# florasion/D-VQVAE

Measured on AMD Instinct MI355X. Metric: grasps/sec at batch=65536, N=1024 pts, K=512, higher is better.
Workload: dtype f32 (GEMMs: every fp32 operand as two fp16 pieces, a1 = fp16(a), a2 = fp16((a - a1) * 2^11), weights pre-scaled by one power of two per output row; the 3 partial products a1 b1, a1 b2, a2 b1 are exact in fp32 and accumulate in TWO fp32 accumulators (large / cross terms) on v_mfma_f32_16x16x32_f16; d

## Files before the change

d-vqvae_amd/_lib.py:

```python
from __future__ import annotations

import ctypes as C
import os
import subprocess
import threading

_HERE = os.path.dirname(os.path.abspath(__file__))
LIB_PATH = os.path.join(_HERE, "libdvq_hip.so")
if os.environ.get("DVQ_DIAG_LIB") == "1":
    LIB_PATH = os.path.join(os.path.dirname(_HERE), "tools", "diag", "libdvq_hip_diag.so")
    print("[dvq] DVQ_DIAG_LIB=1: loading the DIAGNOSTICS build; results are invalid when a DVQ_*_ABL variable is set",
          file=__import__("sys").stderr)
CSRC = os.path.join(_HERE, "csrc")
HEADER = os.path.join(os.path.dirname(_HERE), "include", "dvq.h")

_lock = threading.Lock()
_lib = None

DVQ_MAX_SRC = 8
ABI_VERSION = 10
PLANES_BF16X3, PLANES_F16X2 = 0, 1

c_f32p = C.c_void_p
c_i64p = C.c_void_p
# ... 72 lines not shown
    "dvq_vq_fast_workspace_bytes": (C.c_size_t, [C.c_int64, C.c_int, C.c_int]),
    "dvq_vq_argmin_fast": (C.c_int, [c_f32p, c_f32p, C.c_void_p, C.c_int64, C.c_int, C.c_int, c_i64p, C.c_void_p,
                                     C.c_void_p, C.c_size_t, c_stream]),
    "dvq_vq_lookup": (C.c_int, [c_f32p, c_i64p, C.c_int64, C.c_int64, C.c_int, C.c_int, c_f32p, C.c_int64, c_i32p, c_stream]),
    "dvq_pointnet_workspace_bytes": (C.c_size_t, [C.c_int64, C.c_int]),
    "dvq_pointnet_fault_counters": (C.c_int, [C.POINTER(C.c_uint64), C.c_int]),
    "dvq_pointnet_filter_bytes": (C.c_size_t, []),
    "dvq_pointnet_pack_filter": (C.c_int, [C.c_void_p, C.c_void_p, C.c_void_p, C.c_void_p]),
    "dvq_pointnet_encode": (C.c_int, [C.POINTER(PointnetWeights), c_f32p, C.c_int64, C.c_int, c_f32p, C.c_int64, c_f32p,
                                      C.c_void_p, C.c_size_t, c_stream]),
    "dvq_pixelcnn_tables_bytes": (C.c_size_t, [C.POINTER(PixelcnnWeights)]),
    "dvq_pixelcnn_build_tables": (C.c_int, [C.POINTER(PixelcnnWeights), C.c_void_p, C.c_size_t, c_stream]),
    "dvq_pixelcnn_workspace_bytes": (C.c_size_t, [C.POINTER(PixelcnnWeights), C.c_int64]),
    "dvq_pixelcnn_sample": (C.c_int, [C.POINTER(PixelcnnWeights), c_i64p, c_f32p, C.c_int64, c_i64p, c_f32p, c_i32p,
                                      C.c_void_p, C.c_size_t, c_stream]),
    "dvq_pixelcnn_sample_ctl": (C.c_int, [C.POINTER(PixelcnnWeights), c_i64p, c_f32p, C.c_int64, C.POINTER(PixelcnnCtl), c_i64p, c_f32p,
                                          c_i32p, C.c_void_p, C.c_size_t, c_stream]),
    "dvq_pixelcnn_forward": (C.c_int, [C.POINTER(PixelcnnWeights), c_i64p, c_i64p, C.c_int64, c_f32p, c_i32p, C.c_void_p,
                                       C.c_size_t, c_stream]),
    "dvq_pixelcnn_beam_workspace_bytes": (C.c_size_t, [C.POINTER(PixelcnnWeights), C.c_int64, C.c_int32]),
    "dvq_pixelcnn_beam": (C.c_int, [C.POINTER(PixelcnnWeights), c_i64p, C.c_int64, C.c_int32, c_i64p, c_f32p, c_i32p,
                                    C.POINTER(PixelcnnBeamTrace), c_i32p, C.c_void_p, C.c_size_t, c_stream]),
    "dvq_mano_workspace_bytes": (C.c_size_t, [C.c_int64]),
    "dvq_mano_forward": (C.c_int, [C.POINTER(ManoModel), c_f32p, C.c_int64, c_f32p, C.c_int64, c_f32p, C.c_int64, c_f32p,
                                   C.c_int64, C.c_int64, c_f32p, C.c_int, c_f32p, C.c_void_p, C.c_size_t, c_stream]),
    "dvq_mano_backward_workspace_bytes": (C.c_size_t, [C.c_int64]),
    "dvq_mano_backward": (C.c_int, [C.POINTER(ManoModel), c_f32p, c_f32p, C.c_int64, c_f32p, C.c_int64, c_f32p, C.c_int64, c_f32p,
                                    C.c_int64, C.c_int64, c_f32p, C.c_int, c_f32p, c_f32p, c_f32p, c_f32p, c_f32p, C.c_void_p,
                                    C.c_size_t, c_stream]),
    "dvq_copy_cols": (C.c_int, [c_f32p, C.c_int64, C.c_int64, C.c_int, c_f32p, C.c_int64, c_stream]),
# ... 102 lines not shown
```

d-vqvae_amd/csrc/misc.hip:

```cpp
#include "dvq_internal.h"
#include <string.h>

static thread_local char g_err[512] = "";

void dvq_set_error(const char* fmt, ...) {
    va_list ap;
    va_start(ap, fmt);
    vsnprintf(g_err, sizeof(g_err), fmt, ap);
    va_end(ap);
}

extern "C" const char* dvq_last_error(void) { return g_err; }
extern "C" int dvq_abi_version(void) { return DVQ_ABI_VERSION; }

namespace {
std::mutex g_knob_lock;
std::atomic<const DvqKnobs*> g_knobs{nullptr};
DvqKnobs* read_knobs() {
    DvqKnobs* k = new DvqKnobs();
    auto is = [](const char* name, char c) { const char* e = getenv(name); return e && e[0] == c; };
    auto num = [](const char* name) { const char* e = getenv(name); return e ? atol(e) : 0L; };
    k->gemm_wide = !is("DVQ_GEMM_WIDE", '0');
    k->gemm_tn = (int)num("DVQ_GEMM_TN");
    k->gemm_dephase = !is("DVQ_GEMM_DEPHASE", '0');
// ... 165 lines not shown
    if (b >= B) return;
    const float* src = pc + b * pc_bstride;
    const float x = src[n], y = src[N + n], z = src[2 * N + n];
    const float* r = R + b * 9;
    float* dst = out + b * (long)C * N;
#pragma unroll
    for (int i = 0; i < 3; ++i) {
        float v = r[i * 3 + 0] * x;
        v = fmaf(r[i * 3 + 1], y, v);
        v = fmaf(r[i * 3 + 2], z, v);
        dst[i * N + n] = v + (t ? t[i] : 0.f);
    }
    for (int c = 3; c < C; ++c) dst[c * N + n] = src[c * N + n];
}

__device__ __forceinline__ void philox4x32_10(unsigned (&c)[4], unsigned k0, unsigned k1) {
#pragma unroll
    for (int r = 0; r < 10; ++r) {
        const unsigned long long p0 = (unsigned long long)0xD2511F53u * c[0], p1 = (unsigned long long)0xCD9E8D57u * c[2];
        const unsigned n0 = (unsigned)(p1 >> 32) ^ c[1] ^ k0, n1 = (unsigned)p1, n2 = (unsigned)(p0 >> 32) ^ c[3] ^ k1, n3 = (unsigned)p0;
        c[0] = n0; c[1] = n1; c[2] = n2; c[3] = n3;
        k0 += 0x9E3779B9u;
        k1 += 0xBB67AE85u;
    }
}

__device__ __forceinline__ f32x4 exp1_quad(unsigned long long seed, unsigned stream_id, unsigned long long grow, unsigned q) {
    unsigned c[4] = {q, (unsigned)grow, (unsigned)(grow >> 32), stream_id};
    philox4x32_10(c, (unsigned)seed, (unsigned)(seed >> 32));
    f32x4 v;
#pragma unroll
    for (int i = 0; i < 4; ++i) v[i] = -logf(((float)(c[i] >> 8) + 0.5f) * 5.9604644775390625e-08f);
    return v;
}

__global__ void exp1_noise_kernel(unsigned long long seed, unsigned stream_id, long row0, long rows, int cols, float* __restrict__ out,
                                  const int64_t* __restrict__ perm) {
    const int quads = cols / 4;
    const long gid = (long)blockIdx.x * blockDim.x + threadIdx.x;
    const long r = gid / quads;
    const int q = (int)(gid % quads);
    if (r >= rows) return;
    const unsigned long long grow = (unsigned long long)(row0 + (perm ? (long)perm[r] : r));
    *reinterpret_cast<f32x4*>(out + r * cols + 4 * q) = exp1_quad(seed, stream_id, grow, (unsigned)q);
}

__global__ void exp1_noise_keyed_kernel(unsigned long long seed, const int64_t* __restrict__ stream_ids, const int64_t* __restrict__ row_ids,
                                        long rows, int cols, float* __restrict__ out, int32_t* err_flag) {
    const int quads = cols / 4;
    const long gid = (long)blockIdx.x * blockDim.x + threadIdx.x;
    const long r = gid / quads;
    const int q = (int)(gid % quads);
    if (r >= rows) return;
    const int64_t sid = stream_ids[r], row = row_ids[r];
    f32x4 v;
    if (sid >= 0 && sid <= (int64_t)0xFFFFFFFFLL && row >= 0) {
        v = exp1_quad(seed, (unsigned)sid, (unsigned long long)row, (unsigned)q);
    } else {
        const float nan = __builtin_nanf("");
        v = f32x4{nan, nan, nan, nan};
        if (q == 0 && err_flag) atomicOr(err_flag, 1);
    }
    *reinterpret_cast<f32x4*>(out + r * cols + 4 * q) = v;
}

constexpr int TC_THREADS = 256;
constexpr int TC_SPAN = TC_THREADS * 4;
__device__ __forceinline__ float tc_component(float r0, float r1, float r2, float x, float y, float z, float t) {
    float v = r0 * x;
    v = fmaf(r1, y, v);
    v = fmaf(r2, z, v);
// ... 198 lines not shown
```

d-vqvae_amd/csrc/pixelcnn.hip:

```cpp
#include "dvq_internal.h"

namespace {

constexpr int GRID = 3, NPOS = 9;

__global__ void sanitize_labels_kernel(const int64_t* __restrict__ label, long B, int n_classes, int64_t* __restrict__ out,
                                       int32_t* err_flag) {
    const long b = (long)blockIdx.x * blockDim.x + threadIdx.x;
    if (b >= B) return;
    int64_t l = label[b];
    if (l < 0 || l >= n_classes) {
        if (err_flag) atomicOr(err_flag, 1);
        l = 0;
    }
    out[b] = l;
}

__global__ void bias_gate_kernel(const float* __restrict__ bias, const float* __restrict__ cls, const int64_t* __restrict__ label,
                                 long M, int dim, float* __restrict__ out, float* __restrict__ pre) {
    const long gid = (long)blockIdx.x * blockDim.x + threadIdx.x;
    const long m = gid / dim;
    const int c = (int)(gid % dim);
    if (m >= M) return;
    const int na = (c / 64) * 128 + ((c % 64) / 32) * 64 + (c % 32);
    const int nb = na + 32;
    float a = bias[na], g = bias[nb];
    if (pre) {
        pre[m * 2 * dim + na] = a;
        pre[m * 2 * dim + nb] = g;
    }
    const float* crow = cls + label[m] * 2 * dim;
    a += crow[na];
    g += crow[nb];
    out[m * dim + c] = tanhf(a) * (1.0f / (1.0f + expf(-g)));
}

__global__ void sample_kernel(const float* __restrict__ logits, const float* __restrict__ noise ,
                              int pos, int n_in, long Bc, const int64_t* __restrict__ forced ,
                              int64_t* __restrict__ codes , const float* __restrict__ tok_emb, int dim,
                              float* __restrict__ x0 , float* __restrict__ logits_out ,
                              int32_t* err_flag, const int64_t* __restrict__ lrow ) {
    const int lane = threadIdx.x & 63;
    const long b = (long)blockIdx.x * (blockDim.x >> 6) + (threadIdx.x >> 6);
    if (b >= Bc) return;
    const float* lg = logits + (lrow ? lrow[b] : b) * n_in;
    int64_t code;
    if (logits_out)
        for (int k = lane; k < n_in; k += 64) logits_out[(b * NPOS + pos) * n_in + k] = lg[k];
    if (forced) {
        code = forced[b * NPOS + pos];
        if (code < 0 || code >= n_in) {
            if (lane == 0 && err_flag) atomicOr(err_flag, 1);
            code = 0;
        }
    } else {
        float mx = -INFINITY;
        for (int k = lane; k < n_in; k += 64) mx = fmaxf(mx, lg[k]);
#pragma unroll
        for (int o = 32; o > 0; o >>= 1) mx = fmaxf(mx, __shfl_xor(mx, o));
        float sum = 0.f;
        for (int k = lane; k < n_in; k += 64) sum += expf(lg[k] - mx);
#pragma unroll
        for (int o = 32; o > 0; o >>= 1) sum += __shfl_xor(sum, o);
        const float* q = noise + (b * NPOS + pos) * n_in;
        float best = -INFINITY;
        int bi = 0x7fffffff;
        for (int k = lane; k < n_in; k += 64) {
            const float p = expf(lg[k] - mx) / sum;
            const float s = p / q[k];
            if (s > best || (s == best && k < bi)) { best = s; bi = k; }
        }
#pragma unroll
        for (int o = 32; o > 0; o >>= 1) {
            const float ob = __shfl_xor(best, o);
            const int oi = __shfl_xor(bi, o);
            if (ob > best || (ob == best && oi < bi)) { best = ob; bi = oi; }
        }
        const bool nan_draw = bi == 0x7fffffff;
        if (nan_draw) {
            bi = 0;
            if (lane == 0 && err_flag) atomicOr(err_flag, 4);
        }
        code = bi;
        if (lane == 0) codes[b * NPOS + pos] = nan_draw ? -1 : code;
    }
    const float* e = tok_emb + code * dim;
    for (int c = lane * 4; c < dim; c += 256) *reinterpret_cast<f32x4*>(x0 + b * dim + c) = *reinterpret_cast<const f32x4*>(e + c);
}

__device__ __forceinline__ uint32_t order_key(float v) {
    if (v == 0.f) v = 0.f;
    const uint32_t u = __float_as_uint(v);
    return (u & 0x80000000u) ? ~u : (u | 0x80000000u);
}

__device__ __forceinline__ void row_softmax_stats(const float* __restrict__ lg, int n_in, int lane, float& mx, float& sum) {
    mx = -INFINITY;
    for (int k = lane; k < n_in; k += 64) mx = fmaxf(mx, lg[k]);
#pragma unroll
    for (int o = 32; o > 0; o >>= 1) mx = fmaxf(mx, __shfl_xor(mx, o));
// ... 145 lines not shown
        const float sc = lc / T;
        float lm, ld = code_kept ? (sc - mx) - logf(sum) : -INFINITY;
        if (T == 1.0f && !sel) {
            lm = ld;
        } else {
            float mxl, suml;
            row_softmax_stats(lg, n_in, lane, mxl, suml);
            lm = (lc - mxl) - logf(suml);
        }
        if (nan_row || nan_draw) lm = ld = __builtin_nanf("");
        if (lane == 0) {
            if (logp_model) logp_model[b * NPOS + pos] = lm;
            if (logp_draw) logp_draw[b * NPOS + pos] = ld;
        }
    }
    const float* e = tok_emb + code * dim;
    for (int c = lane * 4; c < dim; c += 256) *reinterpret_cast<f32x4*>(x0 + b * dim + c) = *reinterpret_cast<const f32x4*>(e + c);
}

__global__ void iota_kernel(int64_t* __restrict__ out, int n) {
    const int i = blockIdx.x * blockDim.x + threadIdx.x;
    if (i < n) out[i] = i;
}

__device__ __forceinline__ uint32_t order_key_bits(uint32_t u) {
    if ((u << 1) == 0u) u = 0u;
    return (u & 0x80000000u) ? ~u : (u | 0x80000000u);
}

constexpr int BEAM_MAX_W = 1024, BEAM_THREADS = 1024, BEAM_WAVES = BEAM_THREADS / 64;
// ... 277 lines not shown
int check_weights(const dvq_pixelcnn_weights* w) {
    DVQ_REQUIRE(w && w->layers_host && w->tok_emb && w->w0 && w->b0 && w->w2 && w->b2, "pixelcnn: null weights");
    DVQ_REQUIRE(w->n_layers >= 1 && w->dim >= 64 && w->dim % 64 == 0, "pixelcnn: dim=%d must be a multiple of 64", w->dim);
    DVQ_REQUIRE(w->n_hidden % 32 == 0 && w->n_in >= 1 && w->n_classes >= 1, "pixelcnn: bad head sizes");
    DVQ_REQUIRE(w->planes_kind == DVQ_PLANES_BF16X3 || w->planes_kind == DVQ_PLANES_F16X2, "pixelcnn: unknown planes_kind %d", w->planes_kind);
    if (w->planes_kind == DVQ_PLANES_F16X2 && w->w0_p) {
        DVQ_REQUIRE(w->s0 && w->s2, "pixelcnn: fp16 planes without row scales (head)");
        for (int l = 0; l < w->n_layers; ++l)
            DVQ_REQUIRE(w->layers_host[l].sv && w->layers_host[l].sh && w->layers_host[l].sr, "pixelcnn: fp16 planes without row scales (layer %d)", l);
    }
    return DVQ_OK;
}

int run(const dvq_pixelcnn_weights* w, const int64_t* label, const float* noise, const int64_t* forced, int64_t B,
        int64_t* codes, float* logits_out, int32_t* err_flag, void* ws, size_t ws_bytes, hipStream_t st, void* build = nullptr,
        const dvq_pixelcnn_ctl* ctl = nullptr, const BeamCall* beam = nullptr) {
    DVQ_PROPAGATE(check_weights(w));
    Plan pl;
    if (build) {
        pl = Plan{};
        pl.L = w->n_layers;
        pl.dim = w->dim;
        pl.tab = true;
        (void)carve_tables(pl, w, (char*)build);
    } else {
        DVQ_REQUIRE(B >= 0, "pixelcnn: negative batch");
        if (B == 0) return DVQ_OK;
        DVQ_REQUIRE(label && (beam || forced || (codes && (noise || (ctl && ctl->given)))), "pixelcnn: null input");
        DVQ_REQUIRE(ws && dvq_aligned16(ws), "pixelcnn: null/unaligned workspace");
        pl = make_plan(w, B, ws, beam ? beam->W : 0);
        if (ws_bytes < pl.bytes) {
            dvq_set_error("pixelcnn: workspace %zu < %zu bytes", ws_bytes, pl.bytes);
            return DVQ_EWORKSPACE;
        }
    }
    const int dim = w->dim, L = w->n_layers;
    const int kind = w->planes_kind;

    struct Act { const float* p; const int64_t* arow; };
    auto vertical_layer = [&](int r, int l, long M, const int64_t* lab, auto xv_of ,
                              auto out_of , auto pre_of ,
                              int mode, auto state_of ) -> int {
        const dvq_pixelcnn_layer& ly = w->layers_host[l];
// ... 227 lines not shown
            }
            return Act{pl.XH(level, pos), nullptr};
        };
        for (int r = 0; r < GRID; ++r) {
            cur_r = r;
            cur_pos = r * GRID;
            if (!(pl.tab && r == 0))
                for (int l = 0; l < L; ++l)
                    DVQ_PROPAGATE(vertical_layer(r, l, Bc, pl.lab, xv_b, [&](int c) { return pl.XV(l + 1, r * GRID + c); },
                                                 [&](int c) { return pl.HV(l, c); }, (pl.tab && r == 1 && !beam) ? 2 : 0,
                                                 [&](int c, int which) { return pl.SV(l, c, which); }));
            for (int c = 0; c < GRID; ++c) {
                const int pos = r * GRID + c;
                cur_pos = pos;
                const bool from_table = pl.tab && pos == 0;
                if (!from_table)
                    DVQ_PROPAGATE(horizontal_position(r, c, Bc, pl.lab, [&](int layer, int col) { return hv_b(layer, col, r); }, xh_b,
                                                      [&](int level) { return pl.XH(level, pos); }, pl.g, pl.hid, pl.lg,
                                                      (pl.tab && r == 0 && !beam) ? 2 : 0,
                                                      [&](int layer, int which) { return pl.SH(layer, c, which); }));
                if (beam) {
                    const dvq_pixelcnn_beam_trace* tr = beam->trace;
                    const size_t toff = ((size_t)pos * beam->S + s0) * beam->W;
                    {
                        DVQ_PROF("pixelcnn_beam_score", 0, (double)Bc * 2.0 * w->n_in * 4, st);
                        DVQ_LAUNCH(beam_score_kernel, dim3((unsigned)((Bc + 3) / 4)), dim3(256), 0, st, pl.lg, w->n_in, Bc, beam->W, pl.bscore,
                                   pl.blive, pl.bnan, tr && tr->logits ? tr->logits + toff * w->n_in : nullptr,
                                   from_table ? pl.lgc : nullptr, pl.lab);
                        DVQ_CHECK_LAUNCH("pixelcnn_beam_score");
                    }
// ... 4 lines not shown
                               tr && tr->token ? tr->token + toff : nullptr, tr && tr->score ? tr->score + toff : nullptr,
                               tr && tr->live ? tr->live + (size_t)pos * beam->S + s0 : nullptr);
                    acur ^= 1;
                } else if (ctl) {
                    DVQ_PROF("pixelcnn_draw", 0, (double)Bc * (2.0 * w->n_in + dim) * 4, st);
                    const dim3 grid((unsigned)((Bc + 3) / 4)), block(256);
                    const float* lgp = from_table ? pl.lgc : pl.lg;
                    const float* qp = noise ? noise + b0 * NPOS * w->n_in : nullptr;
                    const int64_t* gp = ctl->given ? ctl->given + b0 * NPOS : nullptr;
                    float* lo = logits_out ? logits_out + b0 * NPOS * w->n_in : nullptr;
                    float* pm = ctl->logp_model_out ? ctl->logp_model_out + b0 * NPOS : nullptr;
                    float* pd = ctl->logp_draw_out ? ctl->logp_draw_out + b0 * NPOS : nullptr;
                    const int64_t* lr = from_table ? pl.lab : nullptr;
                    if (w->n_in <= 512)
                        DVQ_LAUNCH(sample_ctl_kernel<true>, grid, block, 0, st, lgp, qp, pos, w->n_in, Bc, gp, codes + b0 * NPOS, w->tok_emb,
                                   dim, pl.XV(0, pos), lo, err_flag, lr, ctl->temperature, ctl->top_k, pm, pd);
                    else
                        DVQ_LAUNCH(sample_ctl_kernel<false>, grid, block, 0, st, lgp, qp, pos, w->n_in, Bc, gp, codes + b0 * NPOS, w->tok_emb,
                                   dim, pl.XV(0, pos), lo, err_flag, lr, ctl->temperature, ctl->top_k, pm, pd);
                } else {
                DVQ_PROF("pixelcnn_draw", 0, (double)Bc * (2.0 * w->n_in + dim) * 4, st);
                DVQ_LAUNCH(sample_kernel, dim3((unsigned)((Bc + 3) / 4)), dim3(256), 0, st, from_table ? pl.lgc : pl.lg,
                                   noise ? noise + b0 * NPOS * w->n_in : nullptr, pos, w->n_in, Bc,
                                   forced ? forced + b0 * NPOS : nullptr, codes ? codes + b0 * NPOS : nullptr, w->tok_emb, dim,
                                   pl.XV(0, pos), logits_out ? logits_out + b0 * NPOS * w->n_in : nullptr, err_flag,
                                   from_table ? pl.lab : nullptr);
                }
                DVQ_CHECK_LAUNCH("pixelcnn_sample_step");
            }
        }
        if (beam) {
            DVQ_LAUNCH(beam_finish_kernel, dim3((unsigned)((Bc + 255) / 256)), dim3(256), 0, st, pl.btok, pl.anc[acur], pl.chunk, Bc, beam->W,
                       pl.bscore, pl.blive, beam->codes + b0 * NPOS, beam->score + b0, beam->n_live + s0);
            DVQ_CHECK_LAUNCH("pixelcnn_beam_finish");
        }
    }
    return DVQ_OK;
}

}

// ... 9 lines not shown
                "pixelcnn_build_tables: class tables exist for fp16 weight images only (DVQ_PLANES_F16X2)");
    DVQ_REQUIRE(tables_bytes >= dvq_pixelcnn_tables_bytes(w), "pixelcnn_build_tables: buffer %zu < %zu bytes", tables_bytes,
                dvq_pixelcnn_tables_bytes(w));
    return run(w, nullptr, nullptr, nullptr, 0, nullptr, nullptr, nullptr, nullptr, 0, (hipStream_t)stream, tables);
}

extern "C" size_t dvq_pixelcnn_workspace_bytes(const dvq_pixelcnn_weights* w, int64_t B) {
    if (!w || B <= 0) return 256;
    return make_plan(w, B, nullptr).bytes;
}

extern "C" int dvq_pixelcnn_sample(const dvq_pixelcnn_weights* w, const int64_t* label, const float* noise, int64_t B,
                                   int64_t* codes, float* logits_out, int32_t* err_flag, void* workspace,
                                   size_t workspace_bytes, dvq_stream_t stream) {
    return run(w, label, noise, nullptr, B, codes, logits_out, err_flag, workspace, workspace_bytes, (hipStream_t)stream);
}

extern "C" int dvq_pixelcnn_sample_ctl(const dvq_pixelcnn_weights* w, const int64_t* label, const float* noise, int64_t B,
                                       const dvq_pixelcnn_ctl* ctl, int64_t* codes, float* logits_out, int32_t* err_flag,
                                       void* workspace, size_t workspace_bytes, dvq_stream_t stream) {
    DVQ_REQUIRE(ctl, "pixelcnn_sample_ctl: null controls");
    DVQ_REQUIRE(ctl->temperature > 0.f && ctl->temperature <= 3.4028234664e38f, "pixelcnn_sample_ctl: temperature must be finite and > 0");
    DVQ_REQUIRE(ctl->top_k >= 0, "pixelcnn_sample_ctl: top_k must be >= 0 (0: off)");
    DVQ_REQUIRE(codes, "pixelcnn_sample_ctl: null codes");
    return run(w, label, noise, nullptr, B, codes, logits_out, err_flag, workspace, workspace_bytes, (hipStream_t)stream, nullptr, ctl);
}

extern "C" size_t dvq_pixelcnn_beam_workspace_bytes(const dvq_pixelcnn_weights* w, int64_t S, int32_t width) {
    if (!w || S <= 0 || width < 1 || width > BEAM_MAX_W) return 256;
    return make_plan(w, S * width, nullptr, width).bytes;
// ... 23 lines not shown
```

d-vqvae_amd/network/gen_net.py:

```python
import os

import torch
import torch.nn as nn

from .. import _lib, ops, packing
from .DVQVAE import Decoder, _codebooks
from .pixelcnn.models import GatedPixelCNN
from .pointnet_encoder import PointNetEncoder

CODE_SLOTS = ((0, 1), (0, 2), (1, 1), (1, 2), (2, 1), (2, 2))


def code_grid(part_codes, device=None):
    part_codes = torch.as_tensor(part_codes, dtype=torch.int64, device=device)
    if part_codes.dim() != 2 or part_codes.shape[1] != len(CODE_SLOTS):
        raise RuntimeError(f"code_grid: expected [B,{len(CODE_SLOTS)}] part codes, got {tuple(part_codes.shape)}")
    grid = torch.full((part_codes.shape[0], 3, 3), -1, dtype=torch.int64, device=part_codes.device)
    for k, (i, j) in enumerate(CODE_SLOTS):
        grid[:, i, j] = part_codes[:, k]
    return grid


class GenNet(nn.Module):
    def __init__(self, n_embeddings=128, prior_tokens=512, prior_dim=512, prior_layers=15, prior_classes=128):
# ... 50 lines not shown
            seed = dseed if self.noise_seed is None else self.noise_seed
        return seed, (drow if row0 is None else row0), stream_id

    def _draw_noise(self, B, dev, key, perm=None):
        n_in = self.GatedPixelCNN.packed().n_in
        seed, row0, stream_id = key
        return ops.exp1_noise(B, 9 * n_in, seed, row0, stream_id, device=dev, perm=perm).view(B, 9, n_in)

    def _draw_noise_keyed(self, row_keys, seed, err, sel=None):
        n_in = self.GatedPixelCNN.packed().n_in
        sid, rid = row_keys
        if sel is not None:
            sid, rid = sid.index_select(0, sel), rid.index_select(0, sel)
        return ops.exp1_noise_keyed(sid, rid, 9 * n_in, seed, err=err).view(sid.shape[0], 9, n_in)

    def _gen_impl(self, obj, noise, key=None, rows=None, row_keys=None, ctl=None):
        if obj.dim() != 3:
            raise RuntimeError(f"gen: expected obj [B,4,N], got {tuple(obj.shape)}")
        B, dev = obj.shape[0], obj.device
        obj = obj.contiguous()
        z_out = torch.empty(B, 2560, device=dev, dtype=torch.float32)
        z_pos = torch.empty(B, 2048, device=dev, dtype=torch.float32)
        self.obj_encoder_type(obj, out=z_out[:, 1536:])
        self.obj_encoder_pos(obj, out=z_pos[:, 1024:])
        feat_type = z_out[:, 1536:]
        idx6, _ = self.vqvae6.inference(feat_type)
        label = idx6[:, 0].contiguous()
        err = ops.new_err_flag(dev)
        pk = self.GatedPixelCNN.packed()
        logp = None

        def draw(lab, q, given):
            if ctl is None:
                return ops.pixelcnn_sample(pk, lab, q, err=err), None
            c, lm, ld = ops.pixelcnn_sample(pk, lab, q, err=err, temperature=ctl[0], top_k=ctl[1], given=given, return_logp=True)
            return c, (lm, ld)
        given = None if ctl is None else ctl[2]
        if B >= 512 and self.sort_by_label:
            order = torch.argsort(label, stable=True)
            if noise is not None:
                noise_s = noise.index_select(0, order)
            elif row_keys is not None:
                noise_s = self._draw_noise_keyed(row_keys, key, err, sel=order if rows is None else rows.index_select(0, order))
            else:
                noise_s = self._draw_noise(B, dev, key, perm=order if rows is None else rows[order].contiguous())
            codes_s, logp_s = draw(label[order].contiguous(), noise_s, None if given is None else given.index_select(0, order))
            codes = torch.empty_like(codes_s)
            codes[order] = codes_s
            if logp_s is not None:
                logp = tuple(torch.empty_like(t) for t in logp_s)
                for dst, src in zip(logp, logp_s):
                    dst[order] = src
        else:
            if noise is None:
                noise = (self._draw_noise_keyed(row_keys, key, err, sel=rows) if row_keys is not None
                         else self._draw_noise(B, dev, key, perm=rows))
            codes, logp = draw(label, noise.contiguous(), given)
        recon = self._decode(codes.clamp_min(0), {"z_out": z_out}, None, err)
        verts = self._hand_vertices(recon)
        self.recon_encoder(verts, out=z_pos[:, :1024])
        recon_pos = self.pos_decoder(z_pos).view(B, 6)
        aux = dict(idx6=idx6, codes=codes, feat_type=feat_type, feat_pos=z_pos[:, 1024:], verts=verts, hand_feat=z_pos[:, :1024])
        if logp is not None:
            aux["logp_model"], aux["logp_draw"] = logp
        return recon, recon_pos, aux, err

    _RANGE_ERROR = ("GenNet.gen: code or label index out of range (prior classes vs codebook rows, "
                    "gen_net.py:20-34); build GenNet(n_embeddings=...) to match the prior")

    @torch.no_grad()
    def gen(self, obj, noise=None, return_aux=False, seed=None, row0=None, stream_id=None, check=True, row_keys=None,
            temperature=1.0, top_k=0, codes=None, log_prob=False):
# ... 125 lines not shown
```

d-vqvae_amd/ops.py:

```python
from __future__ import annotations

import contextlib
import math
import threading
import ctypes as C
from typing import Dict, List, Optional, Sequence, Tuple

import torch

from . import _lib
from ._lib import check

Tensor = torch.Tensor


def _require_gpu(*ts: Tensor) -> torch.device:
    dev = None
    for t in ts:
        if t is None:
            continue
        if not t.is_cuda:
            raise RuntimeError("dvq ops need tensors on a HIP device (there is no CPU fallback); got " + str(t.device))
        if dev is None:
            dev = t.device
# ... 374 lines not shown
        check(lib.dvq_pointnet_encode(C.byref(packed.cstruct), pc.data_ptr(), B, N, po, ldo,
                                      trans.data_ptr() if want_trans else None, ws.data_ptr(), ws.numel(), _stream(dev)),
              "dvq_pointnet_encode")
    return out, trans


def pointnet_fault_counters(reset: bool = False) -> Tuple[int, int]:
    lib = _lib.load()
    out = (C.c_uint64 * 2)()
    check(lib.dvq_pointnet_fault_counters(out, 1 if reset else 0), "dvq_pointnet_fault_counters")
    return int(out[0]), int(out[1])


def pixelcnn_sample(packed, label: Tensor, noise: Optional[Tensor], return_logits: bool = False, err: Optional[Tensor] = None,
                    _retry: bool = False, temperature: float = 1.0, top_k: int = 0, given: Optional[Tensor] = None,
                    return_logp: bool = False):
    _i64(label, "label")
    if isinstance(temperature, bool) or not isinstance(temperature, (int, float)) or not math.isfinite(temperature) or not temperature > 0:
        raise RuntimeError(f"pixelcnn_sample: temperature must be a finite number > 0, got {temperature!r}")
    if isinstance(top_k, bool) or not isinstance(top_k, int) or top_k < 0:
        raise RuntimeError(f"pixelcnn_sample: top_k must be an integer >= 0 (0: off), got {top_k!r}")
    B = label.shape[0]
    if label.dim() != 1 or not label.is_contiguous():
        raise RuntimeError("pixelcnn_sample: label must be a contiguous [B] tensor")
    if given is not None:
        if (not torch.is_tensor(given) or given.dtype != torch.int64 or tuple(given.shape) not in ((B, 9), (B, 3, 3))
                or not given.is_contiguous() or given.device != label.device):
            raise RuntimeError("pixelcnn_sample: given must be a contiguous int64 [B,9] or [B,3,3] tensor on label's device")
    controlled = float(temperature) != 1.0 or top_k != 0 or given is not None or return_logp
    if noise is None:
        if given is None:
            raise RuntimeError("pixelcnn_sample: noise may be omitted only when given codes are passed")
    else:
        _f32(noise, "noise")
    lib = _lib.load()
    dev = _require_gpu(label, noise, given, err)
    if noise is not None and (tuple(noise.shape) != (B, 9, packed.n_in) or not noise.is_contiguous()):
        raise RuntimeError(f"pixelcnn_sample: noise must be contiguous [B,9,{packed.n_in}], got {tuple(noise.shape)}")
    packed.to(dev)
    codes = torch.empty(B, 3, 3, dtype=torch.int64, device=dev)
    logits = torch.empty(B, 9, packed.n_in, dtype=torch.float32, device=dev) if return_logits else None
    logp = torch.empty(2, B, 9, dtype=torch.float32, device=dev) if return_logp else None
    own_err = err is None
    if own_err:
        err = new_err_flag(dev)
    nws = lib.dvq_pixelcnn_workspace_bytes(C.byref(packed.cstruct), B)
    ws = workspace(nws, dev)
    with torch.cuda.device(dev):
        if not controlled:
            check(lib.dvq_pixelcnn_sample(C.byref(packed.cstruct), label.data_ptr(), noise.data_ptr(), B, codes.data_ptr(),
                                          logits.data_ptr() if return_logits else None, err.data_ptr(), ws.data_ptr(),
                                          ws.numel(), _stream(dev)), "dvq_pixelcnn_sample")
        else:
            ctl = _lib.PixelcnnCtl(float(temperature), int(min(top_k, 2 ** 31 - 1)), given.data_ptr() if given is not None else None,
                                   logp[0].data_ptr() if return_logp else None, logp[1].data_ptr() if return_logp else None)
            check(lib.dvq_pixelcnn_sample_ctl(C.byref(packed.cstruct), label.data_ptr(), noise.data_ptr() if noise is not None else None,
                                              B, C.byref(ctl), codes.data_ptr(), logits.data_ptr() if return_logits else None,
                                              err.data_ptr(), ws.data_ptr(), ws.numel(), _stream(dev)), "dvq_pixelcnn_sample_ctl")
    if own_err:
        e = int(err.item())
        if e & 1:
            raise RuntimeError(f"label or given code out of range for the prior's {packed.n_classes} classes / {packed.n_in} tokens"
                               if controlled else f"label out of range for the prior's {packed.n_classes} classes")
        nan_given = given is not None and not _retry and _out_of_range(packed.kind, logp[0] if return_logp else None, logits)
        if ((e & 4) or nan_given) and packed.kind == _lib.PLANES_F16X2 and not _retry:
            from . import packing
            with packing.gemm_kind_as(_lib.PLANES_BF16X3):
                return pixelcnn_sample(packed, label, noise, return_logits=return_logits, _retry=True, temperature=temperature,
                                       top_k=top_k, given=given, return_logp=return_logp)
    out = (codes,) + ((logits,) if return_logits else ()) + ((logp[0], logp[1]) if return_logp else ())
    return out if len(out) > 1 else codes


PIXELCNN_BEAM_MAX_W = 1024


def pixelcnn_beam(packed, label: Tensor, width: int, trace: bool = False, err: Optional[Tensor] = None):
    if isinstance(width, bool) or not isinstance(width, int) or not 1 <= width <= PIXELCNN_BEAM_MAX_W:
        raise RuntimeError(f"pixelcnn_beam: width must be an integer in 1 .. {PIXELCNN_BEAM_MAX_W}, got {width!r}")
    if not torch.is_tensor(label):
        raise RuntimeError("pixelcnn_beam: label must be a tensor")
    _i64(label, "label")
    if label.dim() != 1 or not label.is_contiguous():
        raise RuntimeError("pixelcnn_beam: label must be a contiguous [S] tensor")
# ... 788 lines not shown
```

include/dvq.h:

```cpp
#ifndef DVQ_H
#define DVQ_H

#include <stddef.h>
#include <stdint.h>

#ifdef __cplusplus
extern "C" {
#endif

typedef void* dvq_stream_t;

typedef enum {
    DVQ_OK = 0,
    DVQ_EINVAL = 1,
    DVQ_EWORKSPACE = 2,
    DVQ_ELAUNCH = 3,
    DVQ_ENODEVICE = 4
} dvq_status;

#define DVQ_ABI_VERSION 10
int dvq_abi_version(void);
const char* dvq_last_error(void);
int dvq_device_count(void);
int dvq_reload_env(void);
// ... 95 lines not shown
    const dvq_pixelcnn_layer* layers_host;
    const float *w0, *b0;
    const float *w2, *b2;
    const uint16_t *w0_p, *w2_p;
    const float *s0, *s2;
    const void* class_tables;
} dvq_pixelcnn_weights;

size_t dvq_pixelcnn_tables_bytes(const dvq_pixelcnn_weights* w_host);
int dvq_pixelcnn_build_tables(const dvq_pixelcnn_weights* w_host, void* tables, size_t tables_bytes, dvq_stream_t stream);

size_t dvq_pixelcnn_workspace_bytes(const dvq_pixelcnn_weights* w_host, int64_t B);
int dvq_pixelcnn_sample(const dvq_pixelcnn_weights* w_host, const int64_t* label, const float* noise,
                        int64_t B, int64_t* codes, float* logits_out, int32_t* err_flag,
                        void* workspace, size_t workspace_bytes, dvq_stream_t stream);
typedef struct {
    float temperature;
    int32_t top_k;
    const int64_t* given;
    float* logp_model_out;
    float* logp_draw_out;
} dvq_pixelcnn_ctl;
int dvq_pixelcnn_sample_ctl(const dvq_pixelcnn_weights* w_host, const int64_t* label, const float* noise,
                            int64_t B, const dvq_pixelcnn_ctl* ctl, int64_t* codes, float* logits_out, int32_t* err_flag,
                            void* workspace, size_t workspace_bytes, dvq_stream_t stream);
int dvq_pixelcnn_forward(const dvq_pixelcnn_weights* w_host, const int64_t* x, const int64_t* label,
                         int64_t B, float* logits , int32_t* err_flag,
                         void* workspace, size_t workspace_bytes, dvq_stream_t stream);
typedef struct {
    int32_t* parent;
// ... 176 lines not shown
```

Baseline: 210,400.

## Generate PixelCNN draw noise inside the sample kernel from Philox keys

Instead of materialising a [B,9,n_in] exponential noise tensor with a separate kernel and reading it back in the sampling kernel, the sample kernel now computes the same Philox-based exp(1) values on the fly from the seed, stream and row keys, spreading quads across lanes with shuffles. This removes the noise buffer's allocation, write and read traffic. The last grid position also skips writing the token embedding, since nothing consumes it. In exchange the draw kernel does extra Philox and log arithmetic per token, and the Python path gains a new keyed API that must reproduce the old noise exactly.

```diff
diff --git a/d-vqvae_amd/_lib.py b/d-vqvae_amd/_lib.py
--- a/d-vqvae_amd/_lib.py
+++ b/d-vqvae_amd/_lib.py
@@ -110,6 +110,10 @@
     "dvq_pixelcnn_workspace_bytes": (C.c_size_t, [C.POINTER(PixelcnnWeights), C.c_int64]),
     "dvq_pixelcnn_sample": (C.c_int, [C.POINTER(PixelcnnWeights), c_i64p, c_f32p, C.c_int64, c_i64p, c_f32p, c_i32p,
                                       C.c_void_p, C.c_size_t, c_stream]),
+    "dvq_pixelcnn_sample_keyed": (C.c_int, [C.POINTER(PixelcnnWeights), c_i64p, C.c_uint64, c_i64p, c_i64p, C.c_int64, c_i64p, c_f32p,
+                                            c_i32p, C.c_void_p, C.c_size_t, c_stream]),
+    "dvq_pixelcnn_sample_stream": (C.c_int, [C.POINTER(PixelcnnWeights), c_i64p, C.c_uint64, C.c_uint32, C.c_int64, c_i64p, C.c_int64,
+                                             c_i64p, c_f32p, c_i32p, C.c_void_p, C.c_size_t, c_stream]),
     "dvq_pixelcnn_sample_ctl": (C.c_int, [C.POINTER(PixelcnnWeights), c_i64p, c_f32p, C.c_int64, C.POINTER(PixelcnnCtl), c_i64p, c_f32p,
                                           c_i32p, C.c_void_p, C.c_size_t, c_stream]),
     "dvq_pixelcnn_forward": (C.c_int, [C.POINTER(PixelcnnWeights), c_i64p, c_i64p, C.c_int64, c_f32p, c_i32p, C.c_void_p,
diff --git a/d-vqvae_amd/csrc/exp1_philox.h b/d-vqvae_amd/csrc/exp1_philox.h
--- /dev/null
+++ b/d-vqvae_amd/csrc/exp1_philox.h
@@ -0,0 +1,26 @@
+#pragma once
+#include "dvq_internal.h"
+
+__device__ __forceinline__ void philox4x32_10(unsigned (&c)[4], unsigned k0, unsigned k1) {
+#pragma unroll
+    for (int r = 0; r < 10; ++r) {
+        const unsigned long long p0 = (unsigned long long)0xD2511F53u * c[0], p1 = (unsigned long long)0xCD9E8D57u * c[2];
+        const unsigned n0 = (unsigned)(p1 >> 32) ^ c[1] ^ k0, n1 = (unsigned)p1, n2 = (unsigned)(p0 >> 32) ^ c[3] ^ k1, n3 = (unsigned)p0;
+        c[0] = n0; c[1] = n1; c[2] = n2; c[3] = n3;
+        k0 += 0x9E3779B9u;
+        k1 += 0xBB67AE85u;
+    }
+}
+
+__device__ __forceinline__ f32x4 exp1_quad(unsigned long long seed, unsigned stream_id, unsigned long long grow, unsigned q) {
+    unsigned c[4] = {q, (unsigned)grow, (unsigned)(grow >> 32), stream_id};
+    philox4x32_10(c, (unsigned)seed, (unsigned)(seed >> 32));
+    f32x4 v;
+#pragma unroll
+    for (int i = 0; i < 4; ++i) v[i] = -logf(((float)(c[i] >> 8) + 0.5f) * 5.9604644775390625e-08f);
+    return v;
+}
+
+__device__ __forceinline__ bool exp1_key_ok(int64_t stream_id, int64_t row_id) {
+    return stream_id >= 0 && stream_id <= (int64_t)0xFFFFFFFFLL && row_id >= 0;
+}
diff --git a/d-vqvae_amd/csrc/misc.hip b/d-vqvae_amd/csrc/misc.hip
--- a/d-vqvae_amd/csrc/misc.hip
+++ b/d-vqvae_amd/csrc/misc.hip
@@ -1,4 +1,5 @@
 #include "dvq_internal.h"
+#include "exp1_philox.h"
 #include <string.h>
 
 static thread_local char g_err[512] = "";
@@ -203,25 +204,6 @@
     for (int c = 3; c < C; ++c) dst[c * N + n] = src[c * N + n];
 }
 
-__device__ __forceinline__ void philox4x32_10(unsigned (&c)[4], unsigned k0, unsigned k1) {
-#pragma unroll
-    for (int r = 0; r < 10; ++r) {
-        const unsigned long long p0 = (unsigned long long)0xD2511F53u * c[0], p1 = (unsigned long long)0xCD9E8D57u * c[2];
-        const unsigned n0 = (unsigned)(p1 >> 32) ^ c[1] ^ k0, n1 = (unsigned)p1, n2 = (unsigned)(p0 >> 32) ^ c[3] ^ k1, n3 = (unsigned)p0;
-        c[0] = n0; c[1] = n1; c[2] = n2; c[3] = n3;
-        k0 += 0x9E3779B9u;
-        k1 += 0xBB67AE85u;
-    }
-}
-
-__device__ __forceinline__ f32x4 exp1_quad(unsigned long long seed, unsigned stream_id, unsigned long long grow, unsigned q) {
-    unsigned c[4] = {q, (unsigned)grow, (unsigned)(grow >> 32), stream_id};
-    philox4x32_10(c, (unsigned)seed, (unsigned)(seed >> 32));
-    f32x4 v;
-#pragma unroll
-    for (int i = 0; i < 4; ++i) v[i] = -logf(((float)(c[i] >> 8) + 0.5f) * 5.9604644775390625e-08f);
-    return v;
-}
 
 __global__ void exp1_noise_kernel(unsigned long long seed, unsigned stream_id, long row0, long rows, int cols, float* __restrict__ out,
                                   const int64_t* __restrict__ perm) {
@@ -243,7 +225,7 @@
     if (r >= rows) return;
     const int64_t sid = stream_ids[r], row = row_ids[r];
     f32x4 v;
-    if (sid >= 0 && sid <= (int64_t)0xFFFFFFFFLL && row >= 0) {
+    if (exp1_key_ok(sid, row)) {
         v = exp1_quad(seed, (unsigned)sid, (unsigned long long)row, (unsigned)q);
     } else {
         const float nan = __builtin_nanf("");
diff --git a/d-vqvae_amd/csrc/pixelcnn.hip b/d-vqvae_amd/csrc/pixelcnn.hip
--- a/d-vqvae_amd/csrc/pixelcnn.hip
+++ b/d-vqvae_amd/csrc/pixelcnn.hip
@@ -1,8 +1,17 @@
 #include "dvq_internal.h"
+#include "exp1_philox.h"
 
 namespace {
 
 constexpr int GRID = 3, NPOS = 9;
+
+struct NoiseKey {
+    unsigned long long seed;
+    const int64_t* stream_ids;
+    const int64_t* row_ids;
+    unsigned stream_id;
+    long row0;
+};
 
 __global__ void sanitize_labels_kernel(const int64_t* __restrict__ label, long B, int n_classes, int64_t* __restrict__ out,
                                        int32_t* err_flag) {
@@ -35,11 +44,13 @@
     out[m * dim + c] = tanhf(a) * (1.0f / (1.0f + expf(-g)));
 }
 
+template <bool KEYED>
 __global__ void sample_kernel(const float* __restrict__ logits, const float* __restrict__ noise ,
                               int pos, int n_in, long Bc, const int64_t* __restrict__ forced ,
                               int64_t* __restrict__ codes , const float* __restrict__ tok_emb, int dim,
                               float* __restrict__ x0 , float* __restrict__ logits_out ,
-                              int32_t* err_flag, const int64_t* __restrict__ lrow ) {
+                              int32_t* err_flag, const int64_t* __restrict__ lrow ,
+                              NoiseKey nk ) {
     const int lane = threadIdx.x & 63;
     const long b = (long)blockIdx.x * (blockDim.x >> 6) + (threadIdx.x >> 6);
     if (b >= Bc) return;
@@ -62,13 +73,48 @@
         for (int k = lane; k < n_in; k += 64) sum += expf(lg[k] - mx);
 #pragma unroll
         for (int o = 32; o > 0; o >>= 1) sum += __shfl_xor(sum, o);
-        const float* q = noise + (b * NPOS + pos) * n_in;
         float best = -INFINITY;
         int bi = 0x7fffffff;
-        for (int k = lane; k < n_in; k += 64) {
-            const float p = expf(lg[k] - mx) / sum;
-            const float s = p / q[k];
-            if (s > best || (s == best && k < bi)) { best = s; bi = k; }
+        if constexpr (KEYED) {
+            const int g = lane >> 2, e = lane & 3;
+            bool key_ok = true;
+            unsigned sid = nk.stream_id;
+            unsigned long long grow;
+            if (nk.stream_ids) {
+                const int64_t ks = nk.stream_ids[b], kr = nk.row_ids[b];
+                key_ok = exp1_key_ok(ks, kr);
+                if (!key_ok && lane == 0 && err_flag) atomicOr(err_flag, 1);
+                sid = (unsigned)ks;
+                grow = (unsigned long long)kr;
+            } else {
+                grow = (unsigned long long)(nk.row0 + (nk.row_ids ? (long)nk.row_ids[b] : b));
+            }
+            const unsigned q0 = (unsigned)(pos * n_in) >> 2;
+            const float nan = __builtin_nanf("");
+            for (int j0 = 0; 64 * j0 < n_in; j0 += 4) {
+                const int jm = j0 + e;
+                f32x4 v = {nan, nan, nan, nan};
+                if (key_ok && 64 * jm + 4 * g < n_in) v = exp1_quad(nk.seed, sid, grow, q0 + 16u * (unsigned)jm + (unsigned)g);
+#pragma unroll
+                for (int r = 0; r < 4; ++r) {
+                    const int cs = (e - r) & 3, t = (e + r) & 3;
+                    const float send = cs == 0 ? v[0] : (cs == 1 ? v[1] : (cs == 2 ? v[2] : v[3]));
+                    const float qk = __shfl(send, (lane & ~3) | t);
+                    const int k = lane + 64 * (j0 + t);
+                    if (k < n_in) {
+                        const float p = expf(lg[k] - mx) / sum;
+                        const float s = p / qk;
+                        if (s > best || (s == best && k < bi)) { best = s; bi = k; }
+                    }
+                }
+            }
+        } else {
+            const float* q = noise + (b * NPOS + pos) * n_in;
+            for (int k = lane; k < n_in; k += 64) {
+                const float p = expf(lg[k] - mx) / sum;
+                const float s = p / q[k];
+                if (s > best || (s == best && k < bi)) { best = s; bi = k; }
+            }
         }
 #pragma unroll
         for (int o = 32; o > 0; o >>= 1) {
@@ -84,6 +130,7 @@
         code = bi;
         if (lane == 0) codes[b * NPOS + pos] = nan_draw ? -1 : code;
     }
+    if (!x0) return;
     const float* e = tok_emb + code * dim;
     for (int c = lane * 4; c < dim; c += 256) *reinterpret_cast<f32x4*>(x0 + b * dim + c) = *reinterpret_cast<const f32x4*>(e + c);
 }
@@ -259,6 +306,7 @@
             if (logp_draw) logp_draw[b * NPOS + pos] = ld;
         }
     }
+    if (!x0) return;
     const float* e = tok_emb + code * dim;
     for (int c = lane * 4; c < dim; c += 256) *reinterpret_cast<f32x4*>(x0 + b * dim + c) = *reinterpret_cast<const f32x4*>(e + c);
 }
@@ -566,7 +614,7 @@
 
 int run(const dvq_pixelcnn_weights* w, const int64_t* label, const float* noise, const int64_t* forced, int64_t B,
         int64_t* codes, float* logits_out, int32_t* err_flag, void* ws, size_t ws_bytes, hipStream_t st, void* build = nullptr,
-        const dvq_pixelcnn_ctl* ctl = nullptr, const BeamCall* beam = nullptr) {
+        const dvq_pixelcnn_ctl* ctl = nullptr, const BeamCall* beam = nullptr, const NoiseKey* nk = nullptr) {
     DVQ_PROPAGATE(check_weights(w));
     Plan pl;
     if (build) {
@@ -578,7 +626,7 @@
     } else {
         DVQ_REQUIRE(B >= 0, "pixelcnn: negative batch");
         if (B == 0) return DVQ_OK;
-        DVQ_REQUIRE(label && (beam || forced || (codes && (noise || (ctl && ctl->given)))), "pixelcnn: null input");
+        DVQ_REQUIRE(label && (beam || forced || (codes && (noise || nk || (ctl && ctl->given)))), "pixelcnn: null input");
         DVQ_REQUIRE(ws && dvq_aligned16(ws), "pixelcnn: null/unaligned workspace");
         pl = make_plan(w, B, ws, beam ? beam->W : 0);
         if (ws_bytes < pl.bytes) {
@@ -836,6 +884,7 @@
                 const int pos = r * GRID + c;
                 cur_pos = pos;
                 const bool from_table = pl.tab && pos == 0;
+                float* x0 = pos == NPOS - 1 ? nullptr : pl.XV(0, pos);
                 if (!from_table)
                     DVQ_PROPAGATE(horizontal_position(r, c, Bc, pl.lab, [&](int layer, int col) { return hv_b(layer, col, r); }, xh_b,
                                                       [&](int level) { return pl.XH(level, pos); }, pl.g, pl.hid, pl.lg,
@@ -870,17 +919,26 @@
                     const int64_t* lr = from_table ? pl.lab : nullptr;
                     if (w->n_in <= 512)
                         DVQ_LAUNCH(sample_ctl_kernel<true>, grid, block, 0, st, lgp, qp, pos, w->n_in, Bc, gp, codes + b0 * NPOS, w->tok_emb,
-                                   dim, pl.XV(0, pos), lo, err_flag, lr, ctl->temperature, ctl->top_k, pm, pd);
+                                   dim, x0, lo, err_flag, lr, ctl->temperature, ctl->top_k, pm, pd);
                     else
                         DVQ_LAUNCH(sample_ctl_kernel<false>, grid, block, 0, st, lgp, qp, pos, w->n_in, Bc, gp, codes + b0 * NPOS, w->tok_emb,
-                                   dim, pl.XV(0, pos), lo, err_flag, lr, ctl->temperature, ctl->top_k, pm, pd);
+                                   dim, x0, lo, err_flag, lr, ctl->temperature, ctl->top_k, pm, pd);
+                } else if (nk) {
+                    NoiseKey key = *nk;
+                    if (key.stream_ids) key.stream_ids += b0;
+                    if (key.row_ids) key.row_ids += b0;
+                    else key.row0 += b0;
+                    DVQ_PROF("pixelcnn_draw", 0, (double)Bc * (w->n_in + dim) * 4, st);
+                    DVQ_LAUNCH(sample_kernel<true>, dim3((unsigned)((Bc + 3) / 4)), dim3(256), 0, st, from_table ? pl.lgc : pl.lg, nullptr, pos,
+                               w->n_in, Bc, nullptr, codes + b0 * NPOS, w->tok_emb, dim, x0,
+                               logits_out ? logits_out + b0 * NPOS * w->n_in : nullptr, err_flag, from_table ? pl.lab : nullptr, key);
                 } else {
-                DVQ_PROF("pixelcnn_draw", 0, (double)Bc * (2.0 * w->n_in + dim) * 4, st);
-                DVQ_LAUNCH(sample_kernel, dim3((unsigned)((Bc + 3) / 4)), dim3(256), 0, st, from_table ? pl.lgc : pl.lg,
-                                   noise ? noise + b0 * NPOS * w->n_in : nullptr, pos, w->n_in, Bc,
-                                   forced ? forced + b0 * NPOS : nullptr, codes ? codes + b0 * NPOS : nullptr, w->tok_emb, dim,
-                                   pl.XV(0, pos), logits_out ? logits_out + b0 * NPOS * w->n_in : nullptr, err_flag,
-                                   from_table ? pl.lab : nullptr);
+                    DVQ_PROF("pixelcnn_draw", 0, (double)Bc * (2.0 * w->n_in + dim) * 4, st);
+                    DVQ_LAUNCH(sample_kernel<false>, dim3((unsigned)((Bc + 3) / 4)), dim3(256), 0, st, from_table ? pl.lgc : pl.lg,
+                               noise ? noise + b0 * NPOS * w->n_in : nullptr, pos, w->n_in, Bc,
+                               forced ? forced + b0 * NPOS : nullptr, codes ? codes + b0 * NPOS : nullptr, w->tok_emb, dim,
+                               x0, logits_out ? logits_out + b0 * NPOS * w->n_in : nullptr, err_flag,
+                               from_table ? pl.lab : nullptr, NoiseKey{});
                 }
                 DVQ_CHECK_LAUNCH("pixelcnn_sample_step");
             }
@@ -920,6 +978,32 @@
                                    int64_t* codes, float* logits_out, int32_t* err_flag, void* workspace,
                                    size_t workspace_bytes, dvq_stream_t stream) {
     return run(w, label, noise, nullptr, B, codes, logits_out, err_flag, workspace, workspace_bytes, (hipStream_t)stream);
+}
+
+static int check_keyed(const dvq_pixelcnn_weights* w, const int64_t* codes, const char* what) {
+    DVQ_REQUIRE(w && codes, "%s: null weights / codes", what);
+    DVQ_REQUIRE(w->n_in % 4 == 0, "%s: n_in=%d must be a multiple of 4", what, w->n_in);
+    return DVQ_OK;
+}
+
+extern "C" int dvq_pixelcnn_sample_keyed(const dvq_pixelcnn_weights* w, const int64_t* label, uint64_t seed, const int64_t* stream_ids,
+                                         const int64_t* row_ids, int64_t B, int64_t* codes, float* logits_out, int32_t* err_flag,
+                                         void* workspace, size_t workspace_bytes, dvq_stream_t stream) {
+    DVQ_PROPAGATE(check_keyed(w, codes, "pixelcnn_sample_keyed"));
+    DVQ_REQUIRE(B <= 0 || (stream_ids && row_ids && err_flag), "pixelcnn_sample_keyed: null keys / error flag");
+    const NoiseKey nk = {seed, stream_ids, row_ids, 0u, 0L};
+    return run(w, label, nullptr, nullptr, B, codes, logits_out, err_flag, workspace, workspace_bytes, (hipStream_t)stream, nullptr, nullptr,
+               nullptr, &nk);
+}
+
+extern "C" int dvq_pixelcnn_sample_stream(const dvq_pixelcnn_weights* w, const int64_t* label, uint64_t seed, uint32_t stream_id, int64_t row0,
+                                          const int64_t* perm, int64_t B, int64_t* codes, float* logits_out, int32_t* err_flag,
+                                          void* workspace, size_t workspace_bytes, dvq_stream_t stream) {
+    DVQ_PROPAGATE(check_keyed(w, codes, "pixelcnn_sample_stream"));
+    DVQ_REQUIRE(row0 >= 0, "pixelcnn_sample_stream: negative row0=%ld", (long)row0);
+    const NoiseKey nk = {seed, nullptr, perm, stream_id, (long)row0};
+    return run(w, label, nullptr, nullptr, B, codes, logits_out, err_flag, workspace, workspace_bytes, (hipStream_t)stream, nullptr, nullptr,
+               nullptr, &nk);
 }
 
 extern "C" int dvq_pixelcnn_sample_ctl(const dvq_pixelcnn_weights* w, const int64_t* label, const float* noise, int64_t B,
diff --git a/d-vqvae_amd/network/gen_net.py b/d-vqvae_amd/network/gen_net.py
--- a/d-vqvae_amd/network/gen_net.py
+++ b/d-vqvae_amd/network/gen_net.py
@@ -88,6 +88,16 @@
             sid, rid = sid.index_select(0, sel), rid.index_select(0, sel)
         return ops.exp1_noise_keyed(sid, rid, 9 * n_in, seed, err=err).view(sid.shape[0], 9, n_in)
 
+    @staticmethod
+    def _draw_key(key, row_keys, sel):
+        if row_keys is not None:
+            sid, rid = row_keys
+            if sel is not None:
+                sid, rid = sid.index_select(0, sel), rid.index_select(0, sel)
+            return (key, sid, rid)
+        seed, row0, stream_id = key
+        return (seed, stream_id, row0) if sel is None else (seed, stream_id, row0, sel.contiguous())
+
     def _gen_impl(self, obj, noise, key=None, rows=None, row_keys=None, ctl=None):
         if obj.dim() != 3:
             raise RuntimeError(f"gen: expected obj [B,4,N], got {tuple(obj.shape)}")
@@ -104,21 +114,24 @@
         pk = self.GatedPixelCNN.packed()
         logp = None
 
-        def draw(lab, q, given):
+        def draw(lab, q, given, qkey=None):
             if ctl is None:
-                return ops.pixelcnn_sample(pk, lab, q, err=err), None
+                return ops.pixelcnn_sample(pk, lab, q, err=err, key=qkey), None
             c, lm, ld = ops.pixelcnn_sample(pk, lab, q, err=err, temperature=ctl[0], top_k=ctl[1], given=given, return_logp=True)
             return c, (lm, ld)
         given = None if ctl is None else ctl[2]
         if B >= 512 and self.sort_by_label:
             order = torch.argsort(label, stable=True)
+            qkey = noise_s = None
             if noise is not None:
                 noise_s = noise.index_select(0, order)
+            elif ctl is None:
+                qkey = self._draw_key(key, row_keys, order if rows is None else rows.index_select(0, order))
             elif row_keys is not None:
                 noise_s = self._draw_noise_keyed(row_keys, key, err, sel=order if rows is None else rows.index_select(0, order))
             else:
                 noise_s = self._draw_noise(B, dev, key, perm=order if rows is None else rows[order].contiguous())
-            codes_s, logp_s = draw(label[order].contiguous(), noise_s, None if given is None else given.index_select(0, order))
+            codes_s, logp_s = draw(label[order].contiguous(), noise_s, None if given is None else given.index_select(0, order), qkey)
             codes = torch.empty_like(codes_s)
             codes[order] = codes_s
             if logp_s is not None:
@@ -126,10 +139,13 @@
                 for dst, src in zip(logp, logp_s):
                     dst[order] = src
         else:
-            if noise is None:
+            qkey = None
+            if noise is None and ctl is None:
+                qkey = self._draw_key(key, row_keys, rows)
+            elif noise is None:
                 noise = (self._draw_noise_keyed(row_keys, key, err, sel=rows) if row_keys is not None
                          else self._draw_noise(B, dev, key, perm=rows))
-            codes, logp = draw(label, noise.contiguous(), given)
+            codes, logp = draw(label, None if noise is None else noise.contiguous(), given, qkey)
         recon = self._decode(codes.clamp_min(0), {"z_out": z_out}, None, err)
         verts = self._hand_vertices(recon)
         self.recon_encoder(verts, out=z_pos[:, :1024])
diff --git a/d-vqvae_amd/ops.py b/d-vqvae_amd/ops.py
--- a/d-vqvae_amd/ops.py
+++ b/d-vqvae_amd/ops.py
@@ -412,7 +412,7 @@
 
 def pixelcnn_sample(packed, label: Tensor, noise: Optional[Tensor], return_logits: bool = False, err: Optional[Tensor] = None,
                     _retry: bool = False, temperature: float = 1.0, top_k: int = 0, given: Optional[Tensor] = None,
-                    return_logp: bool = False):
+                    return_logp: bool = False, key=None):
     _i64(label, "label")
     if isinstance(temperature, bool) or not isinstance(temperature, (int, float)) or not math.isfinite(temperature) or not temperature > 0:
         raise RuntimeError(f"pixelcnn_sample: temperature must be a finite number > 0, got {temperature!r}")
@@ -426,9 +426,28 @@
                 or not given.is_contiguous() or given.device != label.device):
             raise RuntimeError("pixelcnn_sample: given must be a contiguous int64 [B,9] or [B,3,3] tensor on label's device")
     controlled = float(temperature) != 1.0 or top_k != 0 or given is not None or return_logp
-    if noise is None:
+    key_rows = key_perm = None
+    if key is not None:
+        if noise is not None or controlled:
+            raise RuntimeError("pixelcnn_sample: key names the noise of the plain draw; it excludes noise and the draw's controls")
+        if not isinstance(key, tuple) or len(key) not in (3, 4):
+            raise RuntimeError("pixelcnn_sample: key must be (seed, stream_ids, row_ids) or (seed, stream_id, row0[, perm])")
+        if packed.n_in % 4 != 0:
+            raise RuntimeError(f"pixelcnn_sample: a keyed draw needs a token count that is a multiple of 4, got {packed.n_in}")
+        if torch.is_tensor(key[1]):
+            key_rows = key[1:]
+            if len(key) != 3 or not torch.is_tensor(key[2]):
+                raise RuntimeError("pixelcnn_sample: key must be (seed, stream_ids, row_ids) or (seed, stream_id, row0[, perm])")
+        else:
+            key_perm = key[3] if len(key) == 4 else None
+            if int(key[2]) < 0:
+                raise RuntimeError(f"pixelcnn_sample: key row0 must be >= 0, got {key[2]}")
+        for t in (key_rows or ()) + ((key_perm,) if key_perm is not None else ()):
+            if t.dtype != torch.int64 or tuple(t.shape) != (B,) or not t.is_contiguous() or t.device != label.device:
+                raise RuntimeError("pixelcnn_sample: the key's tensors must be contiguous int64 [B] tensors on label's device")
+    elif noise is None:
         if given is None:
-            raise RuntimeError("pixelcnn_sample: noise may be omitted only when given codes are passed")
+            raise RuntimeError("pixelcnn_sample: noise may be omitted only when given codes or a key are passed")
     else:
         _f32(noise, "noise")
     lib = _lib.load()
@@ -445,7 +464,17 @@
     nws = lib.dvq_pixelcnn_workspace_bytes(C.byref(packed.cstruct), B)
     ws = workspace(nws, dev)
     with torch.cuda.device(dev):
-        if not controlled:
+        if key_rows is not None:
+            check(lib.dvq_pixelcnn_sample_keyed(C.byref(packed.cstruct), label.data_ptr(), int(key[0]) & 0xFFFFFFFFFFFFFFFF,
+                                                key_rows[0].data_ptr(), key_rows[1].data_ptr(), B, codes.data_ptr(),
+                                                logits.data_ptr() if return_logits else None, err.data_ptr(), ws.data_ptr(),
+                                                ws.numel(), _stream(dev)), "dvq_pixelcnn_sample_keyed")
+        elif key is not None:
+            check(lib.dvq_pixelcnn_sample_stream(C.byref(packed.cstruct), label.data_ptr(), int(key[0]) & 0xFFFFFFFFFFFFFFFF,
+                                                 int(key[1]) & 0xFFFFFFFF, int(key[2]), key_perm.data_ptr() if key_perm is not None else None,
+                                                 B, codes.data_ptr(), logits.data_ptr() if return_logits else None, err.data_ptr(),
+                                                 ws.data_ptr(), ws.numel(), _stream(dev)), "dvq_pixelcnn_sample_stream")
+        elif not controlled:
             check(lib.dvq_pixelcnn_sample(C.byref(packed.cstruct), label.data_ptr(), noise.data_ptr(), B, codes.data_ptr(),
                                           logits.data_ptr() if return_logits else None, err.data_ptr(), ws.data_ptr(),
                                           ws.numel(), _stream(dev)), "dvq_pixelcnn_sample")
@@ -459,13 +488,14 @@
         e = int(err.item())
         if e & 1:
             raise RuntimeError(f"label or given code out of range for the prior's {packed.n_classes} classes / {packed.n_in} tokens"
-                               if controlled else f"label out of range for the prior's {packed.n_classes} classes")
+                               if controlled else f"label out of range for the prior's {packed.n_classes} classes"
+                               + ("" if key_rows is None else ", or a noise key outside the counter (stream id in [0, 2^32), row id >= 0)"))
         nan_given = given is not None and not _retry and _out_of_range(packed.kind, logp[0] if return_logp else None, logits)
         if ((e & 4) or nan_given) and packed.kind == _lib.PLANES_F16X2 and not _retry:
             from . import packing
             with packing.gemm_kind_as(_lib.PLANES_BF16X3):
                 return pixelcnn_sample(packed, label, noise, return_logits=return_logits, _retry=True, temperature=temperature,
-                                       top_k=top_k, given=given, return_logp=return_logp)
+                                       top_k=top_k, given=given, return_logp=return_logp, key=key)
     out = (codes,) + ((logits,) if return_logits else ()) + ((logp[0], logp[1]) if return_logp else ())
     return out if len(out) > 1 else codes
 
diff --git a/include/dvq.h b/include/dvq.h
--- a/include/dvq.h
+++ b/include/dvq.h
@@ -133,6 +133,12 @@
 int dvq_pixelcnn_sample(const dvq_pixelcnn_weights* w_host, const int64_t* label, const float* noise,
                         int64_t B, int64_t* codes, float* logits_out, int32_t* err_flag,
                         void* workspace, size_t workspace_bytes, dvq_stream_t stream);
+int dvq_pixelcnn_sample_keyed(const dvq_pixelcnn_weights* w_host, const int64_t* label, uint64_t seed,
+                              const int64_t* stream_ids, const int64_t* row_ids, int64_t B, int64_t* codes, float* logits_out,
+                              int32_t* err_flag, void* workspace, size_t workspace_bytes, dvq_stream_t stream);
+int dvq_pixelcnn_sample_stream(const dvq_pixelcnn_weights* w_host, const int64_t* label, uint64_t seed, uint32_t stream_id,
+                               int64_t row0, const int64_t* perm, int64_t B, int64_t* codes, float* logits_out,
+                               int32_t* err_flag, void* workspace, size_t workspace_bytes, dvq_stream_t stream);
 typedef struct {
     float temperature;
     int32_t top_k;
```

Result: no change. 210,900 (median of 6 runs) (+0.2%).
